# JCZ404/Semi-DETR

Hardware: AMD Instinct MI355X
Metric: images/sec/node DINO-R50 SSOD step (hot path: MSDA fwd/bwd + Hungarian + EMA/pseudo-label) (higher is better)
Workload: dtype f32

## Files before the change

semi-detr_amd/csrc/msda.hip:

```cpp
#include <hip/hip_runtime.h>

#include <algorithm>
#include <atomic>
#include <cstdlib>
#include <cstring>
#include <mutex>
#include <type_traits>
#include <vector>

#include "common.h"
#if SEMIDETR_EXPERIMENTS
#include "semidetr_hip_experiments.h"
#endif

#ifndef SEMIDETR_SCATTER_SW
#define SEMIDETR_SCATTER_SW 0
#endif
#ifndef SEMIDETR_SW_NT
#define SEMIDETR_SW_NT 512
#define SEMIDETR_SW_Q 176
#define SEMIDETR_SW_RTH 8
#define SEMIDETR_SW_RTW 16
#define SEMIDETR_SW_WH 24
#define SEMIDETR_SW_WW 32
// ... 318 lines not shown
    const int policy = g_fwd_policy.load(std::memory_order_relaxed);
    use_window = allow_window && policy == 2;
    if (policy != 0 || !allow_window) return SEMIDETR_OK;
    int dev = 0;
    if (hipGetDevice(&dev) != hipSuccess || dev < 0 || dev >= kMaxDevices) return SEMIDETR_OK;
    hipStreamCaptureStatus cap = hipStreamCaptureStatusNone;
    const bool capturing = hipStreamIsCapturing(st, &cap) == hipSuccess && cap != hipStreamCaptureStatusNone;
    std::lock_guard<std::mutex> lock(g_adapt_mu);
    if (!g_adapt[dev]) g_adapt[dev] = new (std::nothrow) FwdAdapt();
    if (!g_adapt[dev]) return SEMIDETR_OK;
    FwdAdapt &a = *g_adapt[dev];
    if (!a.dev_cnt && !a.failed && !capturing) {
        void *h = nullptr, *d = nullptr, *c = nullptr;
        std::vector<unsigned> init((size_t)kPolicySlots * 16, 0u);
        if (hipHostMalloc(&h, kPolicySlots * 16, hipHostMallocMapped) == hipSuccess && hipHostGetDevicePointer(&d, h, 0) == hipSuccess &&
            hipMalloc(&c, kPolicySlots * 64) == hipSuccess) {
            for (int sid = 0; sid < kPolicySlots; ++sid) {
                const unsigned *pp = static_cast<unsigned *>(d) + 4 * sid;
                std::memcpy(&init[(size_t)sid * 16 + 10], &pp, sizeof(pp));
            }
        }
        if (h && d && c && hipMemcpy(c, init.data(), init.size() * sizeof(unsigned), hipMemcpyHostToDevice) == hipSuccess) {
            std::fill_n(static_cast<unsigned *>(h), kPolicySlots * 4, 0u);
            a.pub_host = static_cast<unsigned *>(h);
            a.pub_dev = static_cast<unsigned *>(d);
            a.dev_cnt = static_cast<unsigned *>(c);
        } else {
            (void)hipGetLastError();
            a.failed = true;
        }
    }
    FwdSlot &sl = a.slot[slot_id & (kPolicySlots - 1)];
    if (a.dev_cnt) {
        const int sid = slot_id & (kPolicySlots - 1);
        volatile unsigned *pub = a.pub_host + 4 * sid;
        const unsigned seq = pub[0];
        if (seq != sl.seen_seq) {
            const unsigned far = pub[1], total = pub[2];
            if (pub[0] != seq || far > total) {
            } else if (total) {
                sl.seen_seq = seq;
                sl.last_frac = (float)far / (float)total;
                ++sl.updates;
                if (sl.mode == 0 && sl.last_frac < (levels == 5 ? kFarToWindow5 : kFarToWindow)) sl.mode = 1;
                else if (sl.mode == 1 && sl.last_frac > (levels == 5 ? kFarToPatch5 : kFarToPatch)) sl.mode = 0;
            }
        }
        if (!capturing) {
            const unsigned par = sl.launches++ & 1u;
            unsigned *base = a.dev_cnt + 16 * sid;
            fs = FwdStats{base, par};
        }
    }
    use_window = sl.mode == 1;
    return SEMIDETR_OK;
}

constexpr float kFarToWindowGather = 0.55f;
bool slot_samples_are_near(int slot_id)
{
    const int policy = g_fwd_policy.load(std::memory_order_relaxed);
    if (policy != 0) return policy == 2;
    int dev = 0;
    if (hipGetDevice(&dev) != hipSuccess || dev < 0 || dev >= kMaxDevices) return false;
    std::lock_guard<std::mutex> lock(g_adapt_mu);
    if (!g_adapt[dev]) return false;
    const FwdSlot &sl = g_adapt[dev]->slot[slot_id & (kPolicySlots - 1)];
    return sl.updates > 0 && sl.last_frac >= 0.f && sl.last_frac < kFarToWindowGather;
}

constexpr int kRwProduct4 = rw_tune(kRwWideOffsets | kRwCompact | kRwQueryList | kRwLevelTable | kRwSplitLoad | kRwOneOowPerTrip | kRwLean | kRwOneFine, 2);
constexpr int kRwProduct5 = rw_tune(kRwCompact | kRwQueryList | kRwLevelTable | kRwSplitLoad | kRwRebuildTid | kRwOneOowPerTrip | kRwLean | kRwOneFine, 1);
static_assert(kRwProduct4 == 98320 && kRwProduct5 == 47910, "the product configurations keep their historical numbers");
static_assert(rw_tune_or(kRwProduct4, kRwTailSplit) == 200720, "... and the tail-split variant its own (98320 + 100 x kRwTailSplit)");

template <typename IO, int KL, bool MASK>
struct RwProduct {
    static constexpr bool kRaw = std::is_same<IO, RawIO>::value;
    static_assert((KL == 4 || KL == 5) && (!MASK || kRaw), "four or five levels; the padding mask comes with the fused prologue");
    static constexpr int threads = KL == 4 ? SEMIDETR_RW_NT : SEMIDETR_RW_NT5, rth = KL == 4 ? SEMIDETR_RW_RTH : SEMIDETR_RW_RTH5, rtw = 16;
    static constexpr int hc = KL == 4 ? SEMIDETR_RW_HC : 4, dbg = KL == 4 ? SEMIDETR_RW_DBG : 0, region_px = rth * rtw;
    static constexpr int tune4 = MASK ? SEMIDETR_RW_TUNE_MASK : SEMIDETR_RW_TUNE;
    static constexpr int tune5 = MASK ? SEMIDETR_RW_TUNE5_MASK : (kRaw ? SEMIDETR_RW_TUNE5_RAW : SEMIDETR_RW_TUNE5);
    static constexpr int tune = KL == 5 ? tune5 : (kRaw ? tune4 : rw_tune_spaced(tune4, SEMIDETR_RW_SB_LOCATTN));
    static constexpr int tune_tail = rw_tune_or(tune4, kRwTailSplit);
    template <int TUNE> static constexpr auto kernel_of = &msda_rw_d32<IO, threads, rth, rtw, -1, hc, KL, false, dbg, TUNE, MASK>;
    template <int TUNE> static constexpr size_t lds_of = rw_lds_bytes<threads, rth, rtw, -1, hc, KL, TUNE>();
    static constexpr auto kernel = kernel_of<tune>;
    static constexpr decltype(kernel) kernel_tail = [] {
        if constexpr (KL == 4) return kernel_of<tune_tail>;
        else return decltype(kernel){nullptr};
    }();
    static constexpr size_t lds_bytes = lds_of<tune>;
    static_assert(lds_bytes <= 160 * 1024, "region-window configuration does not fit the LDS");
    static_assert(kernel_tail == nullptr || lds_of<tune_tail> == lds_bytes, "the tail-split instantiation is launched with the same LDS size");
};

template <typename IO>
int launch_fast_forward(hipStream_t st, const float *value, const int64_t *spatial_shapes,
                        const int64_t *level_start, const IO &io, int N, int S, int M, int L, int Lq, int P,
                        int flags, float *out)
{
    SEMIDETR_REQUIRE(!(flags & SEMIDETR_MSDA_QUERIES_ARE_PIXELS) || Lq == S, SEMIDETR_E_BADARG,
                     "msda_forward: SEMIDETR_MSDA_QUERIES_ARE_PIXELS needs num_query == spatial_size");
    const bool pixels = (flags & SEMIDETR_MSDA_QUERIES_ARE_PIXELS) != 0 && (size_t)32 * (L * P + 1) * 32 <= 63 * 1024;
#define LAUNCH_FWD(SP, PT, TILES, LDS)                                                                          \
    hipLaunchKernelGGL((msda_fwd_d32<SP, 4, PT, IO>), dim3((unsigned)((int64_t)N * (TILES) * M)), dim3(256), \
                       (LDS), st, value, spatial_shapes, level_start, io, S, M, L, Lq, P, (TILES), out)
    if (pixels) {
        const bool window_ok = P == kPT && (L == 4 || L == 5) && !(flags & SEMIDETR_MSDA_FIXED_FORWARD) &&
                               (uint64_t)S * M * L * P * 8 < (1ull << 32) && (uint64_t)S * M * kD * 4 < (1ull << 32);
        FwdStats fs;
        bool use_window = false;
        if (int rc = fwd_adapt_next(st, window_ok, (flags >> 8) & 0xff, L, fs, use_window)) return rc;
        if (use_window) {
            bool fell_back = false;
            auto launch_window = [&](auto cfg) -> int {
                using C = decltype(cfg);
                auto kern = C::kernel;
                const auto kern_tail = C::kernel_tail;
                constexpr size_t wlds = C::lds_bytes;
                constexpr int threads = C::threads, region_px = C::region_px;
                const int wbound = ((S * 3 / 4 + region_px - 1) / region_px) * 9 / 8 + 2 * L;
                const int cus = (SEMIDETR_RW_TAIL && kern_tail != nullptr) ? device_cus() : 0;
                const int tail = (int64_t)N * M * ((S * 3 / 4 + region_px - 1) / region_px) < (int64_t)3 * cus ? cus : 0;
                if (tail > 0) kern = kern_tail;
                if (int rc = allow_big_lds(kern, wlds, "msda_forward")) {
                    fell_back = true;
                    return rc;
                }
                SEMIDETR_REQUIRE((int64_t)N * wbound * M + tail < INT32_MAX, SEMIDETR_E_TOOLARGE, "msda_forward: grid too large");
                hipLaunchKernelGGL(kern, dim3((unsigned)((int64_t)N * wbound * M + tail)), dim3(threads), wlds, st, (const float *)nullptr,
                                   value, spatial_shapes, level_start, io, S, M, wbound, out, (float4 *)nullptr, (int64_t)0, fs, tail);
                g_last_kernels = "msda_rw_d32";
                return semidetr::launch_status("msda_rw_d32<forward>");
            };
            auto pick_window = [&]() -> int {
                if constexpr (std::is_same<IO, RawIO>::value) {
                    if (io.has_mask()) return L == 4 ? launch_window(RwProduct<IO, 4, true>{}) : launch_window(RwProduct<IO, 5, true>{});
                }
                return L == 4 ? launch_window(RwProduct<IO, 4, false>{}) : launch_window(RwProduct<IO, 5, false>{});
            };
            const int wrc = pick_window();
            if (!fell_back) return wrc;
            (void)hipGetLastError();
            fs = FwdStats{nullptr, 0u};
        }
        const int bound = (S + 31) / 32 * 5 / 4 + 4 * L;
        SEMIDETR_REQUIRE((int64_t)N * bound * M < INT32_MAX, SEMIDETR_E_TOOLARGE, "msda_forward: grid too large");
        hipLaunchKernelGGL((msda_fwd_d32<1, 4, patch_hw(4, 8), IO>), dim3((unsigned)((int64_t)N * bound * M)), dim3(256),
                           (size_t)32 * (L * P + 1) * 32, st, value, spatial_shapes, level_start, io, S, M, L, Lq, P, bound, out, fs);
        g_last_kernels = "msda_fwd_d32<1, 4, 408";
        return semidetr::launch_status("msda_fwd_d32<patch>");
    }
    int split = pick_split(0, N, Lq, M);
    while (split < 4 && (size_t)(32 / split) * (L * P + 1) * 32 > 64 * 1024) split *= 2;
    const int rpb = 32 / split;
    const int tiles = (Lq + rpb - 1) / rpb;
    SEMIDETR_REQUIRE((int64_t)N * tiles * M < INT32_MAX, SEMIDETR_E_TOOLARGE, "msda_forward: grid too large");
    const size_t lds = (size_t)rpb * (L * P + 1) * 32;
    if (int rc = allow_big_lds(&msda_fwd_d32<4, 4, 0, IO>, lds, "msda_forward")) return rc;
    if (split == 1) LAUNCH_FWD(1, 0, tiles, lds);
    else if (split == 2) LAUNCH_FWD(2, 0, tiles, lds);
    else LAUNCH_FWD(4, 0, tiles, lds);
#undef LAUNCH_FWD
    g_last_kernels = split == 1 ? "msda_fwd_d32<1, 4, 0" : (split == 2 ? "msda_fwd_d32<2, 4, 0" : "msda_fwd_d32<4, 4, 0");
    return semidetr::launch_status("msda_fwd_d32");
}

template <typename IO>
int launch_fast_backward(hipStream_t st, const float *grad_out, const float *value, const int64_t *spatial_shapes,
                         const int64_t *level_start, const IO &io, int N, int S, int M, int L, int Lq, int P,
                         int flags, float *grad_value)
{
    SEMIDETR_REQUIRE(!(flags & SEMIDETR_MSDA_QUERIES_ARE_PIXELS) || Lq == S, SEMIDETR_E_BADARG,
                     "msda_backward: SEMIDETR_MSDA_QUERIES_ARE_PIXELS needs num_query == spatial_size");
    const bool pixels = (flags & SEMIDETR_MSDA_QUERIES_ARE_PIXELS) != 0 && (size_t)32 * (L * P + 1) * 32 <= 63 * 1024;
    const size_t fill = sizeof(float) * (size_t)N * S * M * kD;
    if (pixels && P == kPT && S < (1 << 23) && (uint64_t)S * M * kD * 4 < (1ull << 32) && (uint64_t)S * M * L * P * 8 < (1ull << 32) &&
        (int64_t)M * kD * 4 <= 0xffff) {
#ifndef SEMIDETR_SEPARATE_FILL
#define SEMIDETR_SEPARATE_FILL 0
#endif
        const bool fill_in_gather = !SEMIDETR_SEPARATE_FILL && (L * P == 16 || L * P == 20) && (reinterpret_cast<uintptr_t>(grad_value) & 15) == 0;
        if (!fill_in_gather) {
            const hipError_t e = hipMemsetAsync(grad_value, 0, fill, st);
            if (e != hipSuccess) return semidetr::fail((int)e, "msda_backward memset: %s", hipGetErrorString(e));
        }
        const size_t glds = (size_t)32 * (L * P + 1) * 32 + 2 * kMaxLevels * sizeof(float);
        const int gbound = (S + 31) / 32 * 5 / 4 + 4 * L;
        const int gt = (Lq + 31) / 32;
        SEMIDETR_REQUIRE((int64_t)N * std::max(gbound, gt) * M < INT32_MAX, SEMIDETR_E_TOOLARGE, "msda_backward: grid too large");
        float4 *zero = fill_in_gather ? reinterpret_cast<float4 *>(grad_value) : nullptr;
        bool window_gather = false;
        const bool near = (flags & SEMIDETR_MSDA_GATHER_WINDOW) ? true : ((flags & SEMIDETR_MSDA_GATHER_PATCH) ? false : slot_samples_are_near((flags >> 8) & 0xff));
        if ((L == 4 || L == 5) && P == kPT && (fill_in_gather || SEMIDETR_SEPARATE_FILL) && !(flags & SEMIDETR_MSDA_FIXED_FORWARD) && near &&
            (uint64_t)Lq * M * L * P * 8 < (1ull << 32)) {
            auto launch_gw = [&](auto kern, auto nt_c, size_t wl, int region_px) -> bool {
                constexpr int kGwNT = decltype(nt_c)::value;
                if (allow_big_lds(kern, wl, "msda_backward") != SEMIDETR_OK) {
                    (void)hipGetLastError();
                    return false;
                }
                const int wbound = ((S * 3 / 4 + region_px - 1) / region_px) * 9 / 8 + 2 * L;
                if ((int64_t)N * wbound * M >= INT32_MAX) return false;
                hipLaunchKernelGGL(kern, dim3((unsigned)((int64_t)N * wbound * M)), dim3(kGwNT), wl, st, grad_out, value, spatial_shapes,
                                   level_start, io, S, M, wbound, zero, (int64_t)(fill / 16));
                return true;
            };
            constexpr int kNT5 = std::is_same<IO, RawIO>::value ? SEMIDETR_GW_NT5_RAW : SEMIDETR_GW_NT5;
            constexpr size_t wl4 = gw_lds_bytes<SEMIDETR_GW_NT, SEMIDETR_GW_RTH, SEMIDETR_GW_RTW, SEMIDETR_GW_H0, SEMIDETR_GW_HC, 4>();
            constexpr size_t wl5 = gw_lds_bytes<kNT5, SEMIDETR_GW_RTH5, SEMIDETR_GW_RTW, SEMIDETR_GW_H0, SEMIDETR_GW_HC, 5>();
            constexpr int px4 = SEMIDETR_GW_RTH * SEMIDETR_GW_RTW, px5 = SEMIDETR_GW_RTH5 * SEMIDETR_GW_RTW;
            const std::integral_constant<int, SEMIDETR_GW_NT> nt4;
            const std::integral_constant<int, kNT5> nt5;
            if constexpr (std::is_same<IO, RawIO>::value) {
// ... 378 lines not shown
```

semi-detr_amd/csrc/msda_experiments.h:

```cpp
#pragma once

std::atomic<int> g_fwd_variant_a{0}, g_bwd_variant_a{0};
#define g_fwd_variant (g_fwd_variant_a.load(std::memory_order_relaxed))
#define g_bwd_variant (g_bwd_variant_a.load(std::memory_order_relaxed))

template <typename IO, int NT, int RTH, int RTW, int H0, int HC, int KL, bool GATHER, int DBG = 0, int TUNE = rw_tune(0, 4, 2)>
int launch_rw(hipStream_t st, const float *grad_out, const float *value, const int64_t *spatial_shapes,
              const int64_t *level_start, const IO &io, int N, int S, int M, float *out, float4 *zero, int64_t zero_n4)
{
    auto kern = &msda_rw_d32<IO, NT, RTH, RTW, H0, HC, KL, GATHER, DBG, TUNE>;
    if (int rc = allow_big_lds(kern, rw_lds_bytes<NT, RTH, RTW, H0, HC, KL, TUNE>(), "msda region-window kernel")) return rc;
    const int rpx = RTH * RTW;
    const int bound = ((S * 3 / 4 + rpx - 1) / rpx) * 9 / 8 + 2 * KL;
    const int64_t grid = (int64_t)N * bound * M;
    SEMIDETR_REQUIRE(grid < INT32_MAX, SEMIDETR_E_TOOLARGE, "msda: grid too large");
    constexpr size_t lds = rw_lds_bytes<NT, RTH, RTW, H0, HC, KL, TUNE>();
    static_assert(lds <= 160 * 1024, "region-window configuration does not fit the LDS");
    hipLaunchKernelGGL(kern, dim3((unsigned)grid), dim3(NT), lds, st, grad_out, value, spatial_shapes, level_start, io, S, M,
                       bound, out, zero, zero_n4, FwdStats{nullptr, 0u}, 0);
    return semidetr::launch_status(GATHER ? "msda_rw_d32<gather>" : "msda_rw_d32<forward>");
}

template <typename IO, int KL, bool GATHER>
int launch_rw_cfg(int cfg, hipStream_t st, const float *grad_out, const float *value, const int64_t *spatial_shapes,
                  const int64_t *level_start, const IO &io, int N, int S, int M, float *out, float4 *zero, int64_t zero_n4)
{
#define RW(NT_, RH_, RW_, H0_, HC_) RWT(NT_, RH_, RW_, H0_, HC_, 0, rw_tune(0, 4, 2))
#define RWT(NT_, RH_, RW_, H0_, HC_, DBG_, TUNE_) \
    launch_rw<IO, NT_, RH_, RW_, H0_, HC_, KL, GATHER, DBG_, TUNE_>(st, grad_out, value, spatial_shapes, level_start, io, N, S, M, out, zero, zero_n4)
    constexpr int kLeanFine = kRwLean | kRwOneFine, kRound4 = kRwSplitLoad | kLeanFine;
    if constexpr (KL == 4) {
        switch (cfg) {
        case 0: return RWT(512, 8, 16, 4, 5, 0, rw_tune(0, 4));
        case 1: if constexpr (!GATHER) return RWT(256, 16, 16, -1, 4, 0, rw_tune(0, 4)); else return RWT(512, 8, 16, 4, 5, 0, rw_tune(0, 2));
        case 2: if constexpr (!GATHER) return RWT(512, 16, 16, -1, 4, 0, rw_tune(0, 4)); else return RWT(512, 8, 16, 4, 4, 0, rw_tune(0, 2));
        case 3: if constexpr (!GATHER) return RWT(256, 8, 16, -1, 3, 0, rw_tune(0, 4)); else return RWT(512, 8, 16, 4, 5, 0, rw_tune(0, 6));
        case 4: if constexpr (!GATHER) return RWT(256, 8, 8, -1, 4, 0, rw_tune(0, 4)); else return RWT(768, 24, 16, -1, 5, 0, rw_tune(kRound4, 2));
        case 5: if constexpr (!GATHER) return RWT(256, 8, 16, -1, 4, 0, rw_tune(0, 4)); else return RWT(768, 24, 16, -1, 5, 0, rw_tune(kRound4 | kRwRebuildTid, 2));
        case 6: if constexpr (!GATHER) return RWT(512, 8, 16, -1, 5, 0, rw_tune(0, 4)); else return RWT(768, 16, 16, -1, 6, 0, rw_tune(kRound4, 2));
        case 15: if constexpr (!GATHER) return RWT(512, 16, 16, -1, 5, 0, rw_tune(0, 4)); else break;
        case 16: if constexpr (!GATHER) return RWT(512, 16, 16, -1, 6, 0, rw_tune(0, 4)); else break;
        case 17: if constexpr (!GATHER) return RWT(512, 16, 16, -1, 5, 1, rw_tune(0, 4)); else break;
        case 18: if constexpr (!GATHER) return RWT(512, 16, 16, -1, 6, 0, rw_tune(0, 2)); else break;
        case 19: if constexpr (!GATHER) return RWT(256, 16, 16, -1, 6, 0, rw_tune(0, 2)); else break;
        case 30: if constexpr (!GATHER) return RWT(512, 16, 16, -1, 4, 0, rw_tune(0, 2)); else break;
        case 31: if constexpr (!GATHER) return RWT(1024, 16, 16, -1, 5, 0, rw_tune(kLeanFine | kRwRebuildTid, 2)); else break;
        case 40: if constexpr (!GATHER) return RWT(768, 16, 16, -1, 6, 0, rw_tune(kLeanFine | kRwRebuildTid, 2)); else break;
        case 41: if constexpr (!GATHER) return RWT(1024, 16, 16, -1, 5, 0, rw_tune(kLeanFine | kRwRebuildTid, 1)); else break;
        case 42: if constexpr (!GATHER) return RWT(768, 16, 16, -1, 6, 0, rw_tune(kRound4 | kRwMadU16, 2)); else break;
        case 43: if constexpr (!GATHER) return RWT(768, 16, 16, -1, 6, 0, rw_tune(kRound4, 2)); else break;
        case 44: if constexpr (!GATHER) return RWT(704, 16, 16, -1, 6, 0, rw_tune(kRound4, 2)); else break;
        case 45: if constexpr (!GATHER) return RWT(768, 16, 32, -1, 4, 0, rw_tune(kRound4, 2)); else break;
        case 46: if constexpr (!GATHER) return RWT(704, 16, 32, -1, 5, 0, rw_tune(kRound4, 2)); else break;
        case 47: if constexpr (!GATHER) return RWT(768, 32, 16, -1, 4, 0, rw_tune(kRound4, 2)); else break;
        case 48: if constexpr (!GATHER) return RWT(768, 24, 16, -1, 5, 0, rw_tune(kRound4, 2)); else break;
        case 49: if constexpr (!GATHER) return RWT(704, 32, 16, -1, 5, 0, rw_tune(kRound4, 2)); else break;
        case 51: if constexpr (!GATHER) return RWT(768, 24, 16, -1, 5, 0, rw_tune(kRound4, 2, 1)); else break;
        case 52: if constexpr (!GATHER) return RWT(768, 24, 16, -1, 5, 0, rw_tune(kRound4 | kRwRebuildTid, 2, 1)); else break;
        case 53: if constexpr (!GATHER) return RWT(768, 24, 16, -1, 5, 0, rw_tune(kRound4 | kRwRebuildTid, 2, 2)); else break;
        case 54: if constexpr (!GATHER) return RWT(768, 24, 16, -1, 5, 1, rw_tune(kRound4 | kRwRebuildTid, 2, 1)); else break;
        case 55: if constexpr (!GATHER) return RWT(768, 22, 16, -1, 5, 0, rw_tune(kRound4, 2)); else break;
        case 56: if constexpr (!GATHER) return RWT(768, 25, 16, -1, 5, 0, rw_tune(kRound4, 2)); else break;
        case 57: if constexpr (!GATHER) return RWT(768, 20, 16, -1, 5, 0, rw_tune(kRound4, 2)); else break;
        case 50: if constexpr (!GATHER) return RWT(768, 24, 16, -1, 5, 1, rw_tune(kRound4, 2)); else break;
        case 32: if constexpr (!GATHER) return RWT(512, 16, 16, -1, 6, 0, rw_tune(kRwLean, 2)); else break;
        case 33: if constexpr (!GATHER) return RWT(512, 16, 16, -1, 6, 0, rw_tune(kRwLean, 4)); else break;
        case 34: if constexpr (!GATHER) return RWT(768, 16, 16, -1, 6, 0, rw_tune(kLeanFine, 2)); else break;
        case 35: if constexpr (!GATHER) return RWT(768, 16, 16, -1, 6, 0, rw_tune(kLeanFine, 1)); else break;
        case 36: if constexpr (!GATHER) return RWT(768, 16, 16, -1, 5, 0, rw_tune(kLeanFine, 2)); else break;
        case 37: if constexpr (!GATHER) return RWT(512, 16, 16, -1, 6, 0, rw_tune(kLeanFine, 2)); else break;
        case 38: if constexpr (!GATHER) return RWT(512, 16, 16, -1, 6, 0, rw_tune(kLeanFine, 4)); else break;
        case 39: if constexpr (!GATHER) return RWT(512, 16, 16, -1, 6, 0, rw_tune(kRwOneFine, 2)); else break;
        case 12: if constexpr (!GATHER) return RWT(512, 16, 16, -1, 4, 1, rw_tune(0, 4)); else break;
        case 13: if constexpr (!GATHER) return RWT(512, 16, 16, -1, 4, 2, rw_tune(0, 4)); else break;
        case 14: if constexpr (!GATHER) return RWT(512, 16, 16, -1, 4, 3, rw_tune(0, 4)); else break;
        case 7: if constexpr (!GATHER) return RWT(256, 8, 16, -1, 4, 1, rw_tune(0, 4)); else return RWT(512, 8, 16, 4, 5, 1, rw_tune(0, 4));
        case 8: if constexpr (!GATHER) return RWT(256, 8, 16, -1, 4, 2, rw_tune(0, 4)); else return RWT(512, 8, 16, 4, 5, 2, rw_tune(0, 4));
        case 9: if constexpr (!GATHER) return RWT(256, 8, 16, -1, 4, 3, rw_tune(0, 4)); else return RWT(512, 8, 16, 4, 5, 3, rw_tune(0, 4));
        default: break;
        }
    }
    if constexpr (KL == 5 && !GATHER) {
        if (cfg == 15) return RWT(512, 16, 16, -1, 4, 0, rw_tune(0, 2));
        if (cfg == 18) return RWT(512, 16, 16, -1, 5, 0, rw_tune(0, 2));
        if (cfg == 34) return RWT(768, 16, 16, -1, 4, 0, rw_tune(kLeanFine, 1));
        if (cfg == 35) return RWT(640, 16, 16, -1, 5, 0, rw_tune(kLeanFine, 1));
        if (cfg == 36) return RWT(512, 16, 16, -1, 5, 0, rw_tune(kLeanFine, 2));
        if (cfg == 40) return RWT(768, 16, 16, -1, 4, 0, rw_tune(kLeanFine | kRwRebuildTid, 2));
        if (cfg == 41) return RWT(1024, 16, 16, -1, 4, 0, rw_tune(kLeanFine | kRwRebuildTid, 1));
        if (cfg == 48) return RWT(960, 24, 16, -1, 4, 0, rw_tune(kLeanFine | kRwRebuildTid, 1));
        if (cfg == 49) return RWT(896, 24, 16, -1, 4, 0, rw_tune(kLeanFine | kRwRebuildTid, 1));
    }
    if constexpr (KL == 4) return RWT(512, 8, 16, 4, 5, 0, rw_tune(0, 4));
    else return RWT(512, 8, 16, 4, 4, 0, rw_tune(0, 4));
#undef RWT
#undef RW
}

template <typename IO>
int exp_launch_fast_forward(hipStream_t st, const float *value, const int64_t *spatial_shapes,
                        const int64_t *level_start, const IO &io, int N, int S, int M, int L, int Lq, int P,
                        int flags, float *out)
// ... 594 lines not shown
```

semi-detr_amd/csrc/msda_rw.h:

```cpp
#pragma once

#ifndef SEMIDETR_BRFREE
#define SEMIDETR_BRFREE 1
#endif
constexpr int kRwHeadRun = 16;

enum : int {
    kRwOneFine = 1,
    kRwLean = 2,
    kRwOneOowPerTrip = 4,
    kRwRebuildTid = 8,
    kRwSplitLoad = 16,
    kRwMadU16 = 32,
    kRwLevelTable = 64,
    kRwQueryList = 128,
    kRwCompact = 256,
    kRwWideOffsets = 512,
    kRwTailSplit = 1024,
};
constexpr int rw_tune(int flags, int samples_per_barrier, int preissued = 0) { return 100 * flags + 10 * samples_per_barrier + preissued; }
struct RwTuneFields { int flags, samples_per_barrier, preissued; };
constexpr RwTuneFields rw_untune(int tune) { return RwTuneFields{tune / 100, (tune / 10) % 10, tune % 10}; }
constexpr int rw_tune_or(int tune, int flags) { return rw_tune(rw_untune(tune).flags | flags, rw_untune(tune).samples_per_barrier, rw_untune(tune).preissued); }
constexpr int rw_tune_spaced(int tune, int samples_per_barrier) { return rw_tune(rw_untune(tune).flags, samples_per_barrier, rw_untune(tune).preissued); }
template <int TUNE>
struct RwTune {
    static constexpr int flags = rw_untune(TUNE).flags, samples_per_barrier = rw_untune(TUNE).samples_per_barrier, preissued = rw_untune(TUNE).preissued;
    static constexpr bool one_fine = (flags & kRwOneFine) != 0, lean = (flags & kRwLean) != 0, one_oow_per_trip = (flags & kRwOneOowPerTrip) != 0;
    static constexpr bool rebuild_tid = (flags & kRwRebuildTid) != 0, split_load = (flags & kRwSplitLoad) != 0, mad_u16 = (flags & kRwMadU16) != 0;
    static constexpr bool level_table = (flags & kRwLevelTable) != 0, query_list = (flags & kRwQueryList) != 0, compact = (flags & kRwCompact) != 0;
    static constexpr bool wide = (flags & kRwWideOffsets) != 0, tail = (flags & kRwTailSplit) != 0;
};

template <int RTH, int RTW, int H0, int HC, int KL>
struct RwWin {
    __host__ __device__ static constexpr int ext(int r, int l) { return (r >> l) < 1 ? 1 : (r >> l); }
    __host__ __device__ static constexpr int wh(int l) { return ext(RTH, l) + (l ? 2 * HC + 1 : 2 * H0); }
    __host__ __device__ static constexpr int ww(int l) { return (ext(RTW, l) + (l ? 2 * HC + 1 : 2 * H0)) | 1; }
    static constexpr bool fine_global = H0 < 0;
    __host__ __device__ static constexpr int rows(int l) { return (l == 0 && H0 < 0) ? 0 : wh(l) * ww(l); }
    __host__ __device__ static constexpr int row0(int l)
    {
        int s = 0;
        for (int i = 0; i < l; ++i) s += (rows(i) + 1) & ~1;
        return s;
    }
    __host__ __device__ static constexpr int maxww()
    {
        int w = 0;
        for (int i = (H0 < 0 ? 1 : 0); i < KL; ++i) w = ww(i) > w ? ww(i) : w;
        return w;
    }
    static constexpr int zrow = row0(KL);
    static constexpr int zrows = (maxww() + 2 + 1) & ~1;
    static constexpr int total = zrow + zrows;
};

template <int KL, bool FG = false, bool PRE = false, bool WIDE = false>
constexpr int rw_oct_bytes()
{
    if (WIDE) {
        constexpr int raww = (KL - 1) * kPT * 24 + kPT * 32;
        return raww + (raww % 128 == 0 ? 16 : 0);
    }
    constexpr int raw = FG ? (KL - 1) * kPT * 20 + kPT * 32 + (PRE ? 64 : 0) : KL * kPT * 20 + 64;
    return raw + (raw % 128 == 0 ? 16 : 0);
}

constexpr int kRwQList = 1024;
template <int NT, int RTH, int RTW, int H0, int HC, int KL, int TUNE = 0>
constexpr size_t rw_lds_bytes()
{
    using T = RwTune<TUNE>;
    return (size_t)RwWin<RTH, RTW, H0, HC, KL>::total * 128 + (size_t)(NT / 8) * rw_oct_bytes<KL, (H0 < 0), (T::preissued > 0), T::wide>() +
           (T::level_table ? (size_t)(KL + 1) * 48 : 0) + (T::query_list ? (size_t)kRwQList * 4 : 0);
}

__device__ __forceinline__ int rw_first(int bound, int nq, int nb)
{
    const unsigned long long a = 2ull * (unsigned)nq * (unsigned)bound;
    if (((a + (unsigned)nb) >> 32) == 0) {
        const unsigned cc = ((unsigned)a + (unsigned)nb - 1u) / (unsigned)nb;
        return min(nq, (int)(cc >> 1));
    }
    int lo = 0, hi = nq;
    while (lo < hi) {
        const int mid = lo + ((hi - lo) >> 1);
        if ((2ull * (unsigned)mid + 1ull) * (unsigned)nb >= a) hi = mid;
        else lo = mid + 1;
    }
    return lo;
}

typedef float rw_v2f __attribute__((ext_vector_type(2)));
__device__ __forceinline__ void rw_fma4(float4 &acc, const float4 &w, const float4 &f1, const float4 &f2, const float4 &f3,
                                        const float4 &f4)
{
    rw_v2f a01 = {acc.x, acc.y}, a23 = {acc.z, acc.w};
    const rw_v2f wxy = {w.x, w.y}, wzw = {w.z, w.w};
#define RW_PK_LO(ACC, W, FX, FY) asm("v_pk_fma_f32 %0, %1, %2, %0 op_sel_hi:[0,1,1]" : "+v"(ACC) : "v"(W), "v"(rw_v2f{FX, FY}))
#define RW_PK_HI(ACC, W, FX, FY) asm("v_pk_fma_f32 %0, %1, %2, %0 op_sel:[1,0,0]" : "+v"(ACC) : "v"(W), "v"(rw_v2f{FX, FY}))
    RW_PK_LO(a01, wxy, f1.x, f1.y);
    RW_PK_LO(a23, wxy, f1.z, f1.w);
    RW_PK_HI(a01, wxy, f2.x, f2.y);
    RW_PK_HI(a23, wxy, f2.z, f2.w);
    RW_PK_LO(a01, wzw, f3.x, f3.y);
    RW_PK_LO(a23, wzw, f3.z, f3.w);
    RW_PK_HI(a01, wzw, f4.x, f4.y);
    RW_PK_HI(a23, wzw, f4.z, f4.w);
#undef RW_PK_LO
#undef RW_PK_HI
    acc = make_float4(a01.x, a01.y, a23.x, a23.y);
}

template <typename IO, int NT, int RTH, int RTW, int H0, int HC, int KL, bool GATHER, int DBG = 0, int TUNE = rw_tune(0, 4, 2), bool MASK = false>
__global__ __launch_bounds__(NT, (NT >= 512 ? NT / 256 : 2)) void msda_rw_d32(
    const float *__restrict__ gout, const float *__restrict__ value, const int64_t *__restrict__ shapes,
    const int64_t *__restrict__ starts, const IO io, int S, int M, int regions_bound, float *__restrict__ out,
    float4 *__restrict__ zero, int64_t zero_n4, const FwdStats fs = FwdStats{nullptr, 0u}, int tail_cus = 0)
{
    io.same_dims(S, M, KL);
    using Wn = RwWin<RTH, RTW, H0, HC, KL>;
    constexpr int P = kPT, KLP = KL * P, G = NT / 8, NPASS = (KLP + 7) / 8;
    constexpr bool FG = Wn::fine_global;
    using T = RwTune<TUNE>;
    constexpr bool kWide = T::wide;
    static_assert(!kWide || (FG && !GATHER && T::preissued == 0), "wide window offsets: the forward's product shape");
    constexpr int kOctBytes = rw_oct_bytes<KL, FG, (T::preissued > 0), kWide>();
    constexpr int kRec0 = FG ? P : 0;
    constexpr int kOffAt = (KLP - kRec0) * 16, kFineAt = (KLP - kRec0) * (kWide ? 24 : 20), kSlotAt = (FG && T::preissued > 0) ? kFineAt + P * 32 : kFineAt;
    static_assert(Wn::total * 128 <= (1 << 20), "window offsets are kept in 16 bits, in units of 16 bytes");
    constexpr unsigned kZ0 = (unsigned)Wn::zrow * 128u;
    static_assert(P == 4 && KLP <= 32, "lane j of an octet owns samples j, j + 8, ...");
    static_assert(kOctBytes % 16 == 0, "records are read with ds_read_b128");
    static_assert(!MASK || (FG && !GATHER), "the padding mask is built into the product configuration: forward, level 0 through global loads");

    extern __shared__ float4 smem[];
    char *const lds = reinterpret_cast<char *>(smem);
    char *const recs = lds + Wn::total * 128;
    constexpr bool kTab = T::level_table, kQList = T::query_list, kCompact = T::compact;
    static_assert(!kCompact || (kTab && !GATHER && T::preissued == 0), "compact out-of-window records: forward, level table, nothing pre-issued");
    constexpr bool kLoopAlways = SEMIDETR_BRFREE && kCompact;
    static_assert(!kTab || (T::lean && T::split_load && !GATHER && H0 < 0), "the level table serves the lean forward with split loads");
    int4 *const ltab = reinterpret_cast<int4 *>(recs + (NT / 8) * kOctBytes);
    int *const qlist = reinterpret_cast<int *>(recs + (NT / 8) * kOctBytes + (kTab ? (KL + 1) * 48 : 0));

    const int tid = threadIdx.x, lane = tid & 63;
    const int oc = tid >> 3, j8 = tid & 7;
    const int cls = (tid >> 4) & 1;
    const int Lq = S, rs = M * kD;
    const int b = (int)blockIdx.x;
    unsigned long long tmark = DBG == 1 ? __builtin_readcyclecounter() : 0ull;
    (void)tmark;
    auto lap = [&](int slot_) {
        if (DBG == 1 && tid == 0) {
            const unsigned long long now = __builtin_readcyclecounter();
            SEMIDETR_DBG_ADD(slot_, now - tmark);
            tmark = now;
        }
    };
    unsigned st_far = 0, st_total = 0;

    if (GATHER && zero) {
        const int64_t per = (zero_n4 + gridDim.x - 1) / gridDim.x;
        const int64_t lo = (int64_t)blockIdx.x * per, hi = lo + per < zero_n4 ? lo + per : zero_n4;
        for (int64_t i = lo + tid; i < hi; i += NT) zero[i] = make_float4(0.f, 0.f, 0.f, 0.f);
    }

    const int r_H = lane < KL ? (int)shapes[2 * lane] : 1, r_W = lane < KL ? (int)shapes[2 * lane + 1] : 1;
    const int r_st = lane < KL ? (int)starts[lane] : 0;
    int r_wh = 1, r_ww = 1, r_row0 = 0;
#pragma unroll
    for (int l = 0; l < KL; ++l)
        if (lane == l) { r_wh = Wn::wh(l); r_ww = Wn::ww(l); r_row0 = Wn::row0(l); }
    const int r_H_k = r_H, r_W_k = r_W, r_st_k = r_st, r_wh_k = r_wh, r_ww_k = r_ww, r_row0_k = r_row0;
    int Hs[KL], Ws[KL], sts[KL];
#pragma unroll
    for (int l = 0; l < KL; ++l) {
        Hs[l] = __builtin_amdgcn_readlane(r_H, l);
        Ws[l] = __builtin_amdgcn_readlane(r_W, l);
        sts[l] = __builtin_amdgcn_readlane(r_st, l);
    }
    const int Hb = Hs[0], Wb = Ws[0];
    const int nry = (Hb + RTH - 1) / RTH, nrx = (Wb + RTW - 1) / RTW;

    constexpr bool kTail = !GATHER && T::tail;
    int b_unit = b, part = 0, nparts = 1;
    if (kTail && tail_cus > 0) {
        const int nreg_all = nry * nrx, base_grid = (int)gridDim.x - tail_cus;
        const int nimg = base_grid / (regions_bound * M);
        const int U = nimg * nreg_all * M, full = U / tail_cus * tail_cus, rem = U - full;
        const int s_ = (rem > 0 && regions_bound >= nreg_all && U < 3 * tail_cus) ? min(tail_cus / rem, 4) : 1;
        if (b >= base_grid) {
            const int hidx = b - base_grid;
            if (s_ <= 1 || hidx >= rem * (s_ - 1)) return;
            const int u = full + hidx % rem;
            part = 1 + hidx / rem;
            nparts = s_;
            b_unit = ((u / (nreg_all * M)) * regions_bound + (u / M) % nreg_all) * M + u % M;
        } else {
            const int sl = (b / M) % regions_bound, ni = (b / M) / regions_bound;
            if (s_ > 1 && sl < nreg_all && (ni * nreg_all + sl) * M + b % M >= full) nparts = s_;
        }
    }
    const int m = (b_unit % M + (b_unit / M) / kRwHeadRun) % M;
    const int slot0 = (b_unit / M) % regions_bound, n = (b_unit / M) / regions_bound;
    const bool sampled = !GATHER && fs.on() && (b & 127) == 1 && part == 0;

    const __amdgpu_buffer_rsrc_t vr = image_rsrc(value + (int64_t)n * S * M * kD, (unsigned)S * M * kD * 4u);
    const unsigned lane_b = (unsigned)(m * kD + 4 * j8) * 4u;
    const unsigned row_bytes = (unsigned)rs * 4u;
    constexpr bool kView = !GATHER && kTab;
    const IO iov = kView ? io.image_view(n, Lq, M, KLP) : io;
    float *const out_n = kView ? out + (int64_t)n * Lq * M * kD : out;
    const unsigned char *mask_n = nullptr;
    if constexpr (MASK) mask_n = io.mask + (int64_t)n * S;
    auto mask_of_image = [&]() -> const unsigned char * {
        if constexpr (MASK) {
            int n_ = n;
            asm volatile("" : "+s"(n_));
            return io.mask + (int64_t)n_ * S;
        } else {
            return nullptr;
        }
    };
    int ves[KL];
#pragma unroll
    for (int l = 0; l < KL; ++l) ves[l] = -1;
    if constexpr (MASK) {
        const int r_ve = lane < KL ? io.mask_ext(n, lane).ve : -1;
#pragma unroll
        for (int l = 0; l < KL; ++l) ves[l] = __builtin_amdgcn_readlane(r_ve, l);
    }
    auto ext_vh = [](int ve) { return ve < 0 ? -1 : (ve & 0xffff); };
    auto ext_vw = [](int ve) { return ve < 0 ? -1 : (int)((unsigned)ve >> 16); };

    int myl[NPASS], myH[NPASS], myW[NPASS], myst[NPASS], my_wh1[NPASS], my_ww1[NPASS], my_ww[NPASS], my_row0[NPASS];
#pragma unroll
    for (int p = 0; p < NPASS; ++p) {
        const int l = min((j8 + 8 * p) / P, KL - 1);
        myl[p] = l;
        myH[p] = __shfl(r_H, l, 64);
        myW[p] = __shfl(r_W, l, 64);
        myst[p] = __shfl(r_st, l, 64);
        my_wh1[p] = __shfl(r_wh, l, 64) - 1;
        my_ww[p] = __shfl(r_ww, l, 64);
        my_ww1[p] = my_ww[p] - 1;
        my_row0[p] = __shfl(r_row0, l, 64);
    }

    constexpr bool kLean = T::lean;
    static_assert(!kLean || P == 4, "a pass covers two levels: lanes 0-3 / 4-7");
    struct LvlC { int l, H, W, st, wh1, ww1, ww, row0; };
    auto lvlc = [&](int p) -> LvlC {
        if constexpr (!kLean) {
            return LvlC{myl[p], myH[p], myW[p], myst[p], my_wh1[p], my_ww1[p], my_ww[p], my_row0[p]};
        } else {
            int jj = j8;
            asm volatile("" : "+v"(jj));
            const bool hi = jj >= P;
            const int la = min(2 * p, KL - 1), lb = min(2 * p + 1, KL - 1);
            auto u = [](int v) { return __builtin_amdgcn_readfirstlane(v); };
            return LvlC{hi ? lb : la, hi ? u(Hs[lb]) : u(Hs[la]), hi ? u(Ws[lb]) : u(Ws[la]), hi ? u(sts[lb]) : u(sts[la]),
                        hi ? Wn::wh(lb) - 1 : Wn::wh(la) - 1, hi ? Wn::ww(lb) - 1 : Wn::ww(la) - 1,
                        hi ? Wn::ww(lb) : Wn::ww(la), hi ? Wn::row0(lb) : Wn::row0(la)};
        }
    };

    char *const orec = recs + oc * kOctBytes;
    const char *const wbase = lds + j8 * 16;

    const int Hb_k = Hb, Wb_k = Wb, nrx_k = nrx, nregions = nry * nrx;
    auto run_regions = [&](auto bytes_tag) {
    constexpr bool kBytes = MASK && decltype(bytes_tag)::value;
    for (int reg = slot0; reg < nregions; reg += regions_bound) {
        int Hb_r = Hb_k, Wb_r = Wb_k, nrx_r = nrx_k;
        if (T::rebuild_tid) asm volatile("" : "+s"(Hb_r), "+s"(Wb_r), "+s"(nrx_r));
        const int Hb = Hb_r, Wb = Wb_r, nrx = nrx_r;
        const int nry_b = (Hb + RTH - 1) / RTH, ry_b = reg / nrx, rx_b = reg - ry_b * nrx;
        const int y0b = (ry_b * Hb) / nry_b, y1b = ((ry_b + 1) * Hb) / nry_b;
        const int x0b = (rx_b * Wb) / nrx, x1b = ((rx_b + 1) * Wb) / nrx;
        int lane_t = tid;
        if (T::rebuild_tid) asm volatile("" : "+v"(lane_t));
        const int lane_g = lane_t & 63;
        int g_H = r_H_k, g_W = r_W_k, g_st = r_st_k, g_wh = r_wh_k, g_ww = r_ww_k, g_row0 = r_row0_k;
        if (T::rebuild_tid) {
            g_H = g_W = g_wh = g_ww = 1;
            g_st = g_row0 = 0;
#pragma unroll
            for (int l = 0; l < KL; ++l)
                if (lane_g == l) {
                    g_H = __builtin_amdgcn_readfirstlane(Hs[l]);
                    g_W = __builtin_amdgcn_readfirstlane(Ws[l]);
                    g_st = __builtin_amdgcn_readfirstlane(sts[l]);
                    g_wh = Wn::wh(l);
                    g_ww = Wn::ww(l);
                    g_row0 = Wn::row0(l);
                }
        }
        const int r_H = g_H, r_W = g_W, r_st = g_st, r_wh = g_wh, r_ww = g_ww, r_row0 = g_row0;
        (void)r_row0;
        int r_ylo = 0, r_xlo = 0, r_w = 1, r_cnt = 0;
        float r_invw = 1.f;
        const float pcy = 0.5f * (float)(y0b + y1b) / (float)Hb, pcx = 0.5f * (float)(x0b + x1b) / (float)Wb;
        const int r_wy0 = (int)floorf(pcy * (float)r_H - 0.5f) - r_wh / 2 + 1;
        const int r_wx0 = (int)floorf(pcx * (float)r_W - 0.5f) - r_ww / 2 + 1;
        if (lane < KL) {
            const int ylo_ = rw_first(y0b, r_H, Hb), yhi_ = y1b >= Hb ? r_H : rw_first(y1b, r_H, Hb);
            const int xlo_ = rw_first(x0b, r_W, Wb), xhi_ = x1b >= Wb ? r_W : rw_first(x1b, r_W, Wb);
            r_ylo = ylo_;
            r_xlo = xlo_;
            r_w = max(xhi_ - xlo_, 1);
            r_cnt = max(yhi_ - ylo_, 0) * max(xhi_ - xlo_, 0);
            r_invw = 1.f / (float)r_w;
        }
        int cnt[KL], wy0[KL], wx0[KL], nq_total = 0;
#pragma unroll
        for (int l = 0; l < KL; ++l) {
            cnt[l] = __builtin_amdgcn_readlane(r_cnt, l);
            wy0[l] = __builtin_amdgcn_readlane(r_wy0, l);
            wx0[l] = __builtin_amdgcn_readlane(r_wx0, l);
            nq_total += cnt[l];
        }
        int my_wy0[NPASS], my_wx0[NPASS];
#pragma unroll
        for (int p = 0; p < NPASS; ++p) {
            my_wy0[p] = kLean ? 0 : __shfl(r_wy0, myl[p], 64);
            my_wx0[p] = kLean ? 0 : __shfl(r_wx0, myl[p], 64);
        }
        auto win_origin = [&](int p, int l, int &oy, int &ox) {
            if constexpr (!kLean) {
                oy = my_wy0[p];
                ox = my_wx0[p];
            } else {
                const int la = min(2 * p, KL - 1), lb = min(2 * p + 1, KL - 1);
                oy = l == lb ? __builtin_amdgcn_readfirstlane(wy0[lb]) : __builtin_amdgcn_readfirstlane(wy0[la]);
                ox = l == lb ? __builtin_amdgcn_readfirstlane(wx0[lb]) : __builtin_amdgcn_readfirstlane(wx0[la]);
            }
        };

        const int nrounds_all = (nq_total + G - 1) / G;
        const int round0 = part * nrounds_all / nparts, nrounds = (part + 1) * nrounds_all / nparts;
        auto slot_query = [&](int s) -> int {
            const bool ok = s < nq_total;
            int lq = 0;
#pragma unroll
            for (int l = 0; l < KL - 1; ++l)
                if (lq == l && s >= cnt[l]) { s -= cnt[l]; lq = l + 1; }
            const int yl = __shfl(r_ylo, lq, 64), xl = __shfl(r_xlo, lq, 64), w_ = __shfl(r_w, lq, 64);
            const int st_ = __shfl(r_st, lq, 64), W_ = __shfl(r_W, lq, 64);
            const int dy = (int)(((float)s + 0.5f) * __shfl(r_invw, lq, 64));
            return ok ? st_ + (yl + dy) * W_ + xl + (s - dy * w_) : -1;
        };
        constexpr bool kSplitLoad = T::split_load;
        typename IO::RawXY rr[NPASS];
        float rx[NPASS], ry[NPASS], ra[NPASS];
        float4 go = make_float4(0.f, 0.f, 0.f, 0.f);
        int q = slot_query(round0 * G + (lane_t >> 3));
// ... 556 lines not shown
                            }
                        }
                        const unsigned base = (unsigned)pix * row_bytes + lane_b, wrow = (unsigned)W_ * row_bytes;
                        v2[i][0] = buf_ld4(vr, c_tl ? base : kOob);
                        v2[i][1] = buf_ld4(vr, c_tr ? base + row_bytes : kOob);
                        v2[i][2] = buf_ld4(vr, c_bl ? base + wrow : kOob);
                        v2[i][3] = buf_ld4(vr, c_br ? base + wrow + row_bytes : kOob);
                    }
#pragma unroll
                    for (int i = 0; i < kTrip; ++i)
                        if (act2[i]) consume_fwd(g2[i], v2[i][0], v2[i][1], v2[i][2], v2[i][3]);
                    continue;
                }
#pragma unroll
                for (int i = 0; i < kTrip; ++i) {
                    act2[i] = gmask != 0;
                    k2[i] = act2[i] ? __ffs((int)gmask) - 1 : 0;
                    gmask &= gmask - 1;
                    publish(act2[i], k2[i], i);
                }
                asm volatile("s_waitcnt lgkmcnt(0)" ::: "memory");
                float4 g2[kTrip], v2[kTrip][4];
#pragma unroll
                for (int i = 0; i < kTrip; ++i) {
                    const uint4 o = *reinterpret_cast<const uint4 *>(orec + kSlotAt + 32 * i);
                    g2[i] = *reinterpret_cast<const float4 *>(orec + kSlotAt + 32 * i + 16);
                    v2[i][0] = buf_ld4(vr, (act2[i] ? o.x : kOob) + lane_b);
                    v2[i][1] = buf_ld4(vr, (act2[i] ? o.y : kOob) + lane_b);
                    v2[i][2] = buf_ld4(vr, (act2[i] ? o.z : kOob) + lane_b);
                    v2[i][3] = buf_ld4(vr, (act2[i] ? o.w : kOob) + lane_b);
                }
#pragma unroll
                for (int i = 0; i < kTrip; ++i) {
                    if (!act2[i]) continue;
                    if (!GATHER) {
                        consume_fwd(g2[i], v2[i][0], v2[i][1], v2[i][2], v2[i][3]);
                    } else {
#pragma unroll
                        for (int pp = 0; pp < NPASS; ++pp)
                            if ((k2[i] >> 3) == pp) RW_GATHER_STEP(pp, k2[i] & 7, v2[i][0], v2[i][1], v2[i][2], v2[i][3], g2[i].x, g2[i].y, g2[i].z);
                    }
                }
                asm volatile("s_waitcnt lgkmcnt(0)" ::: "memory");
            }
            lap(8);
            if (DBG == 1 && tid == 0) SEMIDETR_DBG_ADD(10, 1);
            if (!GATHER) {
                if (q_cur >= 0) {
                    if constexpr (kView) st_stream4(out_n + (size_t)((unsigned)(q_cur * M + m) * (unsigned)kD + 4u * (unsigned)j8), acc);
                    else st_stream4(out + (((int64_t)n * Lq + q_cur) * M + m) * kD + 4 * j8, acc);
                }
            } else {
                float dot = 0.f;
                if (IO::kSoftmax) {
#pragma unroll
                    for (int p = 0; p < NPASS; ++p) dot += (j8 + 8 * p < KLP) ? sa[p] * m_a[p] : 0.f;
                    dot = group8_sum(dot);
                }
                if (q_cur >= 0) {
                    const int64_t nq_c = (int64_t)n * Lq + q_cur, row_c = nq_c * M + m;
#pragma unroll
                    for (int p = 0; p < NPASS; ++p) {
                        const int k = j8 + 8 * p;
                        if (k < KLP) {
                            const LvlC c = lvlc(p);
                            const float4 res = make_float4(m_a[p], m_x[p] * (float)c.W, m_y[p] * (float)c.H, sa[p]);
                            io.store_with_dot(row_c, nq_c, KLP, k, c.l, P, c.H, c.W, res, dot);
                        }
                    }
                }
            }
#undef RW_GATHER_STEP
#undef RW_GATHER_DOTS
#undef RW_DOT4
            lap(9);
        }
        if (DBG == 1 && tid == 0) SEMIDETR_DBG_ADD(11, 1);
    }
    };
    if constexpr (MASK && kTab) {
        bool any_bytes = false;
#pragma unroll
        for (int l = 0; l < KL; ++l) any_bytes = any_bytes || ves[l] < 0;
        if (any_bytes) run_regions(std::true_type());
        else run_regions(std::false_type());
    } else if constexpr (MASK) {
        run_regions(std::true_type());
    } else {
        run_regions(std::false_type());
    }
    if (sampled) fwd_stats_add(fs, st_far, st_total, 2u);
    if (!GATHER && fs.on() && b == 0 && tid == 0) fwd_stats_publish(fs);
}
```

Baseline: 452.3.

## Run MSDA region-window forward as persistent workgroups iterating over multiple units

Adds a units mode to the region-window forward kernel. It is enabled by default in the product tune. When the work is large enough, the launch uses about one workgroup per CU instead of one per (image, region, head). Each workgroup walks a strided list of (image, region, head) units, rebuilding the value resource, IO view, output pointer and mask extents whenever the image changes. This is meant to cut workgroup launch and tail overhead and amortise per-workgroup setup, at the cost of per-unit recomputation, less latency hiding from oversubscription, and more complex mask handling.

```diff
diff --git a/semi-detr_amd/csrc/msda.hip b/semi-detr_amd/csrc/msda.hip
--- a/semi-detr_amd/csrc/msda.hip
+++ b/semi-detr_amd/csrc/msda.hip
@@ -424,7 +424,8 @@
     static constexpr int hc = KL == 4 ? SEMIDETR_RW_HC : 4, dbg = KL == 4 ? SEMIDETR_RW_DBG : 0, region_px = rth * rtw;
     static constexpr int tune4 = MASK ? SEMIDETR_RW_TUNE_MASK : SEMIDETR_RW_TUNE;
     static constexpr int tune5 = MASK ? SEMIDETR_RW_TUNE5_MASK : (kRaw ? SEMIDETR_RW_TUNE5_RAW : SEMIDETR_RW_TUNE5);
-    static constexpr int tune = KL == 5 ? tune5 : (kRaw ? tune4 : rw_tune_spaced(tune4, SEMIDETR_RW_SB_LOCATTN));
+    static constexpr int tune_one = KL == 5 ? tune5 : (kRaw ? tune4 : rw_tune_spaced(tune4, SEMIDETR_RW_SB_LOCATTN));
+    static constexpr int tune = rw_tune_or(tune_one, kRwUnits);
     static constexpr int tune_tail = rw_tune_or(tune4, kRwTailSplit);
     template <int TUNE> static constexpr auto kernel_of = &msda_rw_d32<IO, threads, rth, rtw, -1, hc, KL, false, dbg, TUNE, MASK>;
     template <int TUNE> static constexpr size_t lds_of = rw_lds_bytes<threads, rth, rtw, -1, hc, KL, TUNE>();
@@ -465,15 +466,19 @@
                 constexpr int threads = C::threads, region_px = C::region_px;
                 const int wbound = ((S * 3 / 4 + region_px - 1) / region_px) * 9 / 8 + 2 * L;
                 const int cus = (SEMIDETR_RW_TAIL && kern_tail != nullptr) ? device_cus() : 0;
-                const int tail = (int64_t)N * M * ((S * 3 / 4 + region_px - 1) / region_px) < (int64_t)3 * cus ? cus : 0;
+                const int64_t units_hint = (int64_t)N * M * ((S * 3 / 4 + region_px - 1) / region_px);
+                const int tail = units_hint < (int64_t)3 * cus ? cus : 0;
                 if (tail > 0) kern = kern_tail;
+                const int all_cus = device_cus();
+                const bool multi = tail == 0 && all_cus > 0 && units_hint >= (int64_t)3 * all_cus;
+                const int64_t grid = tail > 0 ? (int64_t)N * wbound * M + tail : (multi ? (int64_t)msda_units_grid(all_cus) : (int64_t)N * wbound * M);
                 if (int rc = allow_big_lds(kern, wlds, "msda_forward")) {
                     fell_back = true;
                     return rc;
                 }
                 SEMIDETR_REQUIRE((int64_t)N * wbound * M + tail < INT32_MAX, SEMIDETR_E_TOOLARGE, "msda_forward: grid too large");
-                hipLaunchKernelGGL(kern, dim3((unsigned)((int64_t)N * wbound * M + tail)), dim3(threads), wlds, st, (const float *)nullptr,
-                                   value, spatial_shapes, level_start, io, S, M, wbound, out, (float4 *)nullptr, (int64_t)0, fs, tail);
+                hipLaunchKernelGGL(kern, dim3((unsigned)grid), dim3(threads), wlds, st, (const float *)nullptr,
+                                   value, spatial_shapes, level_start, io, S, M, wbound, out, (float4 *)nullptr, (int64_t)0, fs, tail, N);
                 g_last_kernels = "msda_rw_d32";
                 return semidetr::launch_status("msda_rw_d32<forward>");
             };
diff --git a/semi-detr_amd/csrc/msda_experiments.h b/semi-detr_amd/csrc/msda_experiments.h
--- a/semi-detr_amd/csrc/msda_experiments.h
+++ b/semi-detr_amd/csrc/msda_experiments.h
@@ -12,12 +12,13 @@
     if (int rc = allow_big_lds(kern, rw_lds_bytes<NT, RTH, RTW, H0, HC, KL, TUNE>(), "msda region-window kernel")) return rc;
     const int rpx = RTH * RTW;
     const int bound = ((S * 3 / 4 + rpx - 1) / rpx) * 9 / 8 + 2 * KL;
-    const int64_t grid = (int64_t)N * bound * M;
-    SEMIDETR_REQUIRE(grid < INT32_MAX, SEMIDETR_E_TOOLARGE, "msda: grid too large");
+    const int cus = RwTune<TUNE>::units ? device_cus() : 0;
+    const int64_t grid = cus > 0 ? (int64_t)msda_units_grid(cus) : (int64_t)N * bound * M;
+    SEMIDETR_REQUIRE((int64_t)N * bound * M < INT32_MAX, SEMIDETR_E_TOOLARGE, "msda: grid too large");
     constexpr size_t lds = rw_lds_bytes<NT, RTH, RTW, H0, HC, KL, TUNE>();
     static_assert(lds <= 160 * 1024, "region-window configuration does not fit the LDS");
     hipLaunchKernelGGL(kern, dim3((unsigned)grid), dim3(NT), lds, st, grad_out, value, spatial_shapes, level_start, io, S, M,
-                       bound, out, zero, zero_n4, FwdStats{nullptr, 0u}, 0);
+                       bound, out, zero, zero_n4, FwdStats{nullptr, 0u}, 0, N);
     return semidetr::launch_status(GATHER ? "msda_rw_d32<gather>" : "msda_rw_d32<forward>");
 }
 
diff --git a/semi-detr_amd/csrc/msda_rw.h b/semi-detr_amd/csrc/msda_rw.h
--- a/semi-detr_amd/csrc/msda_rw.h
+++ b/semi-detr_amd/csrc/msda_rw.h
@@ -3,7 +3,8 @@
 #ifndef SEMIDETR_BRFREE
 #define SEMIDETR_BRFREE 1
 #endif
-constexpr int kRwHeadRun = 16;
+#include "msda_units.h"
+constexpr int kRwHeadRun = kMsdaHeadRun;
 
 enum : int {
     kRwOneFine = 1,
@@ -17,6 +18,7 @@
     kRwCompact = 256,
     kRwWideOffsets = 512,
     kRwTailSplit = 1024,
+    kRwUnits = 2048,
 };
 constexpr int rw_tune(int flags, int samples_per_barrier, int preissued = 0) { return 100 * flags + 10 * samples_per_barrier + preissued; }
 struct RwTuneFields { int flags, samples_per_barrier, preissued; };
@@ -29,7 +31,7 @@
     static constexpr bool one_fine = (flags & kRwOneFine) != 0, lean = (flags & kRwLean) != 0, one_oow_per_trip = (flags & kRwOneOowPerTrip) != 0;
     static constexpr bool rebuild_tid = (flags & kRwRebuildTid) != 0, split_load = (flags & kRwSplitLoad) != 0, mad_u16 = (flags & kRwMadU16) != 0;
     static constexpr bool level_table = (flags & kRwLevelTable) != 0, query_list = (flags & kRwQueryList) != 0, compact = (flags & kRwCompact) != 0;
-    static constexpr bool wide = (flags & kRwWideOffsets) != 0, tail = (flags & kRwTailSplit) != 0;
+    static constexpr bool wide = (flags & kRwWideOffsets) != 0, tail = (flags & kRwTailSplit) != 0, units = (flags & kRwUnits) != 0;
 };
 
 template <int RTH, int RTW, int H0, int HC, int KL>
@@ -117,7 +119,7 @@
 __global__ __launch_bounds__(NT, (NT >= 512 ? NT / 256 : 2)) void msda_rw_d32(
     const float *__restrict__ gout, const float *__restrict__ value, const int64_t *__restrict__ shapes,
     const int64_t *__restrict__ starts, const IO io, int S, int M, int regions_bound, float *__restrict__ out,
-    float4 *__restrict__ zero, int64_t zero_n4, const FwdStats fs = FwdStats{nullptr, 0u}, int tail_cus = 0)
+    float4 *__restrict__ zero, int64_t zero_n4, const FwdStats fs = FwdStats{nullptr, 0u}, int tail_cus = 0, int nimg = 0)
 {
     io.same_dims(S, M, KL);
     using Wn = RwWin<RTH, RTW, H0, HC, KL>;
@@ -203,9 +205,19 @@
             if (s_ > 1 && sl < nreg_all && (ni * nreg_all + sl) * M + b % M >= full) nparts = s_;
         }
     }
-    const int m = (b_unit % M + (b_unit / M) / kRwHeadRun) % M;
-    const int slot0 = (b_unit / M) % regions_bound, n = (b_unit / M) / regions_bound;
-    const bool sampled = !GATHER && fs.on() && (b & 127) == 1 && part == 0;
+    constexpr bool kUnits = T::units;
+    static_assert(!kUnits || (!GATHER && !T::tail), "multi-unit workgroups: the forward, without the tail split's helper workgroups");
+    int m = (b_unit % M + (b_unit / M) / kRwHeadRun) % M;
+    int slot0 = (b_unit / M) % regions_bound, n = (b_unit / M) / regions_bound;
+    unsigned unit_index = (unsigned)b;
+    if constexpr (kUnits) {
+        const MsdaUnit u0 = msda_unit(b, 0, nimg, M, nry * nrx, (int)gridDim.x);
+        if (u0.n < 0) return;
+        n = u0.n;
+        m = u0.m;
+        slot0 = u0.region;
+    }
+    bool sampled = !GATHER && fs.on() && (unit_index & 127u) == 1u && part == 0;
 
     const __amdgpu_buffer_rsrc_t vr = image_rsrc(value + (int64_t)n * S * M * kD, (unsigned)S * M * kD * 4u);
     const unsigned lane_b = (unsigned)(m * kD + 4 * j8) * 4u;
@@ -225,12 +237,16 @@
         }
     };
     int ves[KL];
+    int r_ve_unit = -1;
 #pragma unroll
     for (int l = 0; l < KL; ++l) ves[l] = -1;
     if constexpr (MASK) {
         const int r_ve = lane < KL ? io.mask_ext(n, lane).ve : -1;
 #pragma unroll
         for (int l = 0; l < KL; ++l) ves[l] = __builtin_amdgcn_readlane(r_ve, l);
+        r_ve_unit = r_ve;
+        if constexpr (T::units)
+            if (nimg * KL <= 64) r_ve_unit = lane < nimg * KL ? io.mask_ext(lane / KL, lane - (lane / KL) * KL).ve : -1;
     }
     auto ext_vh = [](int ve) { return ve < 0 ? -1 : (ve & 0xffff); };
     auto ext_vw = [](int ve) { return ve < 0 ? -1 : (int)((unsigned)ve >> 16); };
@@ -273,7 +289,52 @@
     const int Hb_k = Hb, Wb_k = Wb, nrx_k = nrx, nregions = nry * nrx;
     auto run_regions = [&](auto bytes_tag) {
     constexpr bool kBytes = MASK && decltype(bytes_tag)::value;
-    for (int reg = slot0; reg < nregions; reg += regions_bound) {
+    int unit_k = 0;
+    auto next_region = [&](int reg) -> int {
+        if constexpr (!kUnits) {
+            return reg + regions_bound;
+        } else {
+            const MsdaUnit u = msda_unit(b, ++unit_k, nimg, M, nregions, (int)gridDim.x);
+            if (u.n < 0) return nregions;
+            if (u.n != n) {
+                n = u.n;
+                if constexpr (MASK) {
+                    if (nimg * KL > 64) {
+                        const int ln = (int)__builtin_amdgcn_mbcnt_hi(~0u, __builtin_amdgcn_mbcnt_lo(~0u, 0u));
+                        r_ve_unit = ln < KL ? io.mask_ext(n, ln).ve : -1;
+                    }
+                }
+            }
+            m = u.m;
+            sampled = fs.on() && (u.index & 127u) == 1u;
+            return u.region;
+        }
+    };
+    const auto &vr_k = vr;
+    const IO &iov_k = iov;
+    float *const out_k = out_n;
+    const unsigned char *const mask_k = mask_n;
+    const int(&ves_k)[KL] = ves;
+    for (int reg = slot0; reg < nregions; reg = next_region(reg)) {
+        auto unit_vr = [&]() -> __amdgpu_buffer_rsrc_t {
+            if constexpr (kUnits) return image_rsrc(value + (int64_t)n * S * M * kD, (unsigned)S * M * kD * 4u);
+            else return vr_k;
+        };
+        auto unit_io = [&]() -> IO {
+            if constexpr (kUnits && kView) return io.image_view(n, Lq, M, KLP);
+            else return iov_k;
+        };
+        auto unit_out = [&]() -> float * {
+            if constexpr (kUnits && kView) return out + (int64_t)n * Lq * M * kD;
+            else return out_k;
+        };
+        const __amdgpu_buffer_rsrc_t vr = unit_vr();
+        const IO iov = unit_io();
+        float *const out_n = unit_out();
+        const unsigned char *const mask_n = (kUnits && MASK) ? mask_of_image() : mask_k;
+        int ves[KL];
+#pragma unroll
+        for (int l = 0; l < KL; ++l) ves[l] = (kUnits && MASK) ? __builtin_amdgcn_readlane(r_ve_unit, (nimg * KL <= 64 ? n * KL : 0) + l) : ves_k[l];
         int Hb_r = Hb_k, Wb_r = Wb_k, nrx_r = nrx_k;
         if (T::rebuild_tid) asm volatile("" : "+s"(Hb_r), "+s"(Wb_r), "+s"(nrx_r));
         const int Hb = Hb_r, Wb = Wb_r, nrx = nrx_r;
@@ -996,6 +1057,11 @@
         bool any_bytes = false;
 #pragma unroll
         for (int l = 0; l < KL; ++l) any_bytes = any_bytes || ves[l] < 0;
+        if constexpr (kUnits) {
+            bool mine = false;
+            for (int i = lane; i < nimg * KL; i += 64) mine = mine || io.mask_ext(i / KL, i - (i / KL) * KL).ve < 0;
+            any_bytes = __any(mine);
+        }
         if (any_bytes) run_regions(std::true_type());
         else run_regions(std::false_type());
     } else if constexpr (MASK) {
@@ -1003,6 +1069,6 @@
     } else {
         run_regions(std::false_type());
     }
-    if (sampled) fwd_stats_add(fs, st_far, st_total, 2u);
+    if (kUnits ? (!GATHER && fs.on()) : sampled) fwd_stats_add(fs, st_far, st_total, 2u);
     if (!GATHER && fs.on() && b == 0 && tid == 0) fwd_stats_publish(fs);
 }
diff --git a/semi-detr_amd/csrc/msda_units.h b/semi-detr_amd/csrc/msda_units.h
--- /dev/null
+++ b/semi-detr_amd/csrc/msda_units.h
@@ -0,0 +1,38 @@
+#pragma once
+
+#if defined(__HIPCC__) || defined(__CUDACC__)
+#define MSDA_UNITS_HD __host__ __device__ __forceinline__
+#else
+#define MSDA_UNITS_HD inline
+#endif
+
+constexpr int kMsdaHeadRun = 16;
+
+struct MsdaUnit {
+    int n, region, m;
+    unsigned index;
+};
+
+MSDA_UNITS_HD unsigned long long msda_unit_count(int N, int M, int nregions)
+{
+    return (unsigned long long)(N > 0 ? N : 0) * (unsigned)(M > 0 ? M : 0) * (unsigned)(nregions > 0 ? nregions : 0);
+}
+
+MSDA_UNITS_HD MsdaUnit msda_unit(int workgroup, int k, int N, int M, int nregions, int G)
+{
+    const unsigned long long units = msda_unit_count(N, M, nregions);
+    const unsigned long long u64 = (unsigned long long)(unsigned)workgroup + (unsigned long long)(unsigned)k * (unsigned)G;
+    if (workgroup < 0 || k < 0 || G <= 0 || workgroup >= G || u64 >= units || units > 0x7fffffffull) return MsdaUnit{-1, 0, 0, 0u};
+    const unsigned u = (unsigned)u64, pair = u / (unsigned)M, h = u - pair * (unsigned)M;
+    const unsigned n = pair / (unsigned)nregions;
+    return MsdaUnit{(int)n, (int)(pair - n * (unsigned)nregions), (int)((h + pair / (unsigned)kMsdaHeadRun) % (unsigned)M), u};
+}
+
+MSDA_UNITS_HD unsigned msda_units_of_workgroup(int workgroup, int N, int M, int nregions, int G)
+{
+    const unsigned long long units = msda_unit_count(N, M, nregions);
+    if (workgroup < 0 || G <= 0 || workgroup >= G || (unsigned long long)workgroup >= units) return 0u;
+    return (unsigned)((units - (unsigned)workgroup + (unsigned)G - 1u) / (unsigned)G);
+}
+
+MSDA_UNITS_HD int msda_units_grid(int cus) { return cus >= 8 ? cus & ~7 : (cus > 0 ? cus : 1); }
```

Measured after the change: 456.7 (median of 6 runs). No clear change (+1.0%).
